# line/open-universe

Hardware: AMD Instinct MI355X
Metric: real_time_factor (audio s / wall s), UNIVERSE++ 16 kHz 8-step enhance (higher is better)
Workload: dtype f32; 1 GPU; UNIVERSE++ 16 kHz, 8 diffusion steps, batch=1 utterance(s) of 4 s per GPU per step; network=PP16, n_diffusion_steps=8, batch_per_gpu=1, samples_per_utterance=64000, launches_per_enhance=414

## Files before the change

### open-universe_amd/csrc/ou_api.cpp

```cpp
#include <hip/hip_runtime.h>

#include <cmath>
#include <cstdio>
#include <cstdlib>
#include <cstring>
#include <map>
#include <string>
#include <vector>

#include "../../include/ouniverse.h"
#include "../../include/ouniverse_tuning.h"
#include "ou_kernels.h"
#include "ou_model.h"

using namespace ou;

namespace {
thread_local std::string g_last_error;
constexpr int kMaxSteps = 256;
constexpr size_t kProfSlots = 32768;
constexpr float kInvSqrt2 = 0.70710678118654752440f;
constexpr size_t align256(size_t bytes) { return (bytes + 255) & ~size_t(255); }

struct TensorRef {
  size_t off;
  int C, T;
};
struct Options {
  int dbg = 0, xcd_map = -1, conv_direct = 5, fuse = -1, fuse_nc = 0, rate_small = 1, fuse_upfir = 1, block3 = 0, d4_fir = 1,
      d4_force = 0, d4_short = 1, d2_wk = 0, wino = 1, d2_map = -1, unfuse64 = 0, preact = 1;
  int gru_v = 2, gru_bmax = 0, gru_ts = 0, gru_upw = 0, gru_backoff = 0, gru_agent = -1, gru_dbg = 0;
  int split = -1;
  int dbg_dec0_under_gru = 0;
  int tile_prefetch = 1;
  int trace = 0, no_overlap = 0, ts = 0, deep_factor = 8, mask_fused = 1, split_wino = 1, d2_tile_rule = 1;
  int ens_share = 1;
  double tile_min = -1.0;
  std::string chain_ts;
};
}

struct ou_packer {
  Model m;
  std::map<std::string, HostTensor> sd;
  std::vector<float> blob;
  std::string err;
};

struct ou_handle {
  Model m;
  const float* W = nullptr;
  int device = 0;
  int num_cu = 256;
  std::string err;
  std::map<std::string, TensorRef> tensors;
  int n_launch = 0, n_conv = 0;
  int cond_B = 0, cond_T = 0;
  bool trace = false;
  Options opt;
  NormMode norm;
  std::string plan_with_options;
  int last_cfg = -1;
  long long* tstamps = nullptr;
  std::map<size_t, float> alphas;
  hipStream_t aux[3] = {nullptr, nullptr, nullptr};
  std::vector<hipEvent_t> events;
  size_t ev_used = 0;
  bool overlap = true;
  int force_cfg = -1, force_sc = 0;
  bool profile = false;
  struct ProfRec { double flops, bytes; int cfg; };
  std::vector<ProfRec> prof;
  size_t prof_used = 0;
  unsigned long long* prof_dev = nullptr;
  struct WsRec { const void* ws; size_t bytes; int B, T; };
  std::vector<WsRec> ws_ready;
  int gru_agent_stores = 0;
  int lanes = 1, lane = 0;
  int lane_max_b = 0;
  struct NoiseSource {
    bool on = false;
    unsigned long long seed = 0;
    std::vector<unsigned long long> streams;
    float* scratch = nullptr;
    size_t scratch_bytes = 0;
  } noise_src;
  double plane_per_sample = 0.0, wav_plane_per_sample = 0.0;
  bool ws_ok(const void* ws, size_t bytes, int B, int T) const {
    (void)T;
    for (const WsRec& r : ws_ready)
      if (r.ws == ws) return r.B == B && r.bytes <= bytes;
    return false;
  }
};

namespace {

int fail(ou_handle* h, int code, const std::string& msg) {
  if (h) h->err = msg;
  g_last_error = msg;
  return code;
}

struct Tensor {
  float* p = nullptr;
  int C = 0, T = 0;
};

struct OptDesc {
  const char* key;
  int Options::*ip;
  double Options::*dp;
  bool experiments_only;
  const char* doc;
};
const OptDesc kOptions[] = {
    {"conv_direct", &Options::conv_direct, nullptr, false, "kernel generations the conv launcher may use (0 .. 5, ConvArgs::direct)"},
    {"split", &Options::split, nullptr, false, "-1 rule / 0 never / 1 wherever possible: conv_split_kernel (bf16-split operands)"},
    {"split_wino", &Options::split_wino, nullptr, false, "experiments build: 0 = the plain bf16-split kernel also where its minimal-filtering form would take the layer"},
    {"wino", &Options::wino, nullptr, false, "0: never the minimal-filtering (Winograd / Cook-Toom) kernel variants"},
    {"fuse", &Options::fuse, nullptr, false, "-1 cost model / 0 never / 2 / 3: depth of the fused ConvBlock body (conv_chain kernels)"},
    {"fuse_nc", &Options::fuse_nc, nullptr, false, "128 / 256: columns per tile of the fused ConvBlock body (0: launcher's choice)"},
    {"fuse_upfir", &Options::fuse_upfir, nullptr, false, "0: up-path anti-alias FIR always as its own pass"},
    {"rate_small", &Options::rate_small, nullptr, false, "0: outermost rate-change convs on the generic kernels (no rate_down / rate_up)"},
    {"preact", &Options::preact, nullptr, false, "0: every PReLU in its consumer's operand path (ConvArgs::out_act never set)"},
    {"unfuse64", &Options::unfuse64, nullptr, false, "1: 64-channel ConvBlock bodies as three split-K launches"},
    {"block3", &Options::block3, nullptr, false, "1: the three body convs of a deep-level ConvBlock in one launch (experiments build only)"},
    {"xcd_map", &Options::xcd_map, nullptr, false, "block -> tile mapping of the LDS-tiled conv kernel (-1: launcher's choice)"},
    {"d2_map", &Options::d2_map, nullptr, false, "block -> tile mapping of the wide-load split-K kernels (-1: launcher's choice)"},
    {"d2_tile_rule", &Options::d2_tile_rule, nullptr, false, "0: round 5's 64- vs 32-column rule of the wide-load split-K kernels (ignores that only 64-column tiles have minimal filtering)"},
    {"d2_wk", &Options::d2_wk, nullptr, false, "4 / 8: K slices of conv_direct2_kernel (0: launcher's rule)"},
    {"d4_fir", &Options::d4_fir, nullptr, false, "0: up convs with a fusable FIR stay on the first-generation fused kernel"},
    {"d4_short", &Options::d4_short, nullptr, false, "0: the 401-frame levels at batch 1 stay on the first-generation kernels"},
    {"d4_force", &Options::d4_force, nullptr, false, "10 TM + log2(WK): that conv_direct4 tile shape wherever a layer admits it"},
    {"tile_min", nullptr, &Options::tile_min, false, "wave tiles per SIMD from which the no-split-K kernels take a layer (< 0: 1.2)"},
    {"tile_prefetch", &Options::tile_prefetch, nullptr, false, "0: no LDS prefetch of the epilogue operand in conv_direct3_kernel"},
    {"deep_factor", &Options::deep_factor, nullptr, false, "blocks of 64 x 128 per CU up to which a layer counts as 'deep' (split-K kernels)"},
    {"mask_fused", &Options::mask_fused, nullptr, false, "ragged batches: 0 = a separate tail-mask launch after EVERY producer (reference form of the masks)"},
    {"gru_v", &Options::gru_v, nullptr, false, "2 ring kernel / 1 polling-wave kernel (experiments build)"},
    {"gru_bmax", &Options::gru_bmax, nullptr, false, "cap on the utterances per GRU launch (forces the chunked path)"},
    {"gru_upw", &Options::gru_upw, nullptr, false, "hidden units per workgroup of the ring kernel (0: from the batch size)"},
    {"gru_backoff", &Options::gru_backoff, nullptr, false, "poll back-off experiments of the ring kernel (0: none)"},
    {"gru_agent_stores", &Options::gru_agent, nullptr, false, "-1 handle's mode / 0 plain / 1 agent-scope publishes"},
    {"gru_dbg", &Options::gru_dbg, nullptr, false, "bit 0 no republish safety net, bit 1 system-scope publishes, bit 2 FAULT INJECTION (tests)"},
    {"gru_ts", &Options::gru_ts, nullptr, false, "1: per-wave cycle stamps of the GRU kernel into the end of the workspace (tuning)"},
    {"ts", &Options::ts, nullptr, false, "1: per-wave phase stamps in ou_bench_conv (tuning)"},
    {"trace", &Options::trace, nullptr, false, "1: one line per conv launch on stderr"},
    {"no_overlap", &Options::no_overlap, nullptr, false, "1: no side streams inside a call (every kernel alone on the device)"},
    {"ens_share", &Options::ens_share, nullptr, false, "ou_enhance_ensemble: 1 = conditioner once over the B inputs, its results replicated; 0 = over all E * B rows"},
    {"dbg", &Options::dbg, nullptr, true, "phase ablation switches of the conv kernels: WRONG results by design"},
    {"dbg_dec0", &Options::dbg_dec0_under_gru, nullptr, true, "first decoder block under the GRU: upper-bound measurement, WRONG results"},
};
constexpr int kNumOptions = (int)(sizeof(kOptions) / sizeof(kOptions[0]));
const OptDesc* find_option(const char* key) {
  for (int i = 0; i < kNumOptions; i++)
    if (std::strcmp(kOptions[i].key, key) == 0) return &kOptions[i];
  return nullptr;
}

struct Runner {
  ou_handle* h;
  Options env;
  char* base;
  size_t cap;
  size_t off = 0;
  bool dry;
  hipStream_t st;
  hipStream_t main_st;
  int B;
  hipError_t herr = hipSuccess;
  bool oom = false;
  const char* where = "";
  size_t max_plane = 0;
  bool mel_scale_preset = false;
  bool ragged = false;
  const int* lens_dev = nullptr;
  const RowInfo* rows_dev = nullptr;
  LevelSpec lv;
  int level_T[kMaxLenLevels] = {0};
  unsigned* status_words = nullptr;
  unsigned long long* block3_bar = nullptr;
  int gru_area_rows = 0;
  bool gru_shared = false;

  Runner(ou_handle* h_, void* ws, size_t cap_, bool dry_, hipStream_t st_, int B_)
      : h(h_), env(h_->opt), base((char*)ws), cap(cap_), dry(dry_), st(st_), main_st(st_), B(B_) {
#ifndef OU_EXPERIMENTS
    env.dbg = 0; env.dbg_dec0_under_gru = 0;
#endif
  }
  static Runner conditioner_of(const Runner& r, int Bc) {
    Runner c(r.h, r.base, r.cap, false, r.st, Bc);
    c.status_words = r.status_words;
    c.block3_bar = r.block3_bar;
    c.gru_area_rows = r.B;
    c.off = r.off;
    c.mel_scale_preset = r.mel_scale_preset;
    c.lv = r.lv;
    for (int l = 0; l < kMaxLenLevels; l++) c.level_T[l] = r.level_T[l];
    return c;
  }
  void set_ragged(const int* lens, const RowInfo* rows) {
    ragged = true;
    lens_dev = lens;
    rows_dev = rows;
  }

  bool ok() const { return herr == hipSuccess && !oom; }
  template <class F>
  void launch(const char* w, F&& enqueue) {
    if (dry || !ok()) return;
    chk(enqueue(), w);
  }

  float* alloc_raw(size_t floats) {
    size_t bytes = align256(floats * 4);
    size_t o = off;
    off += bytes;
    if (!dry && off > cap) { oom = true; return (float*)base; }
    return dry ? nullptr : (float*)(base + o);
  }
  Tensor alloc(const std::string& name, int C, int T) {
    size_t o = off;
    Tensor t;
    t.p = alloc_raw((size_t)B * C * T);
    if ((size_t)C * T * 4 > max_plane) max_plane = (size_t)C * T * 4;
    t.C = C;
    t.T = T;
    if (!name.empty()) h->tensors[name] = TensorRef{o, C, T};
    return t;
  }
  hipEvent_t next_event() {
    if (h->ev_used == h->events.size()) {
      hipEvent_t e;
      if (hipEventCreateWithFlags(&e, hipEventDisableTiming) != hipSuccess) return nullptr;
      h->events.push_back(e);
    }
    return h->events[h->ev_used++];
  }
  void wait_for(hipStream_t from, hipStream_t to, const char* w_record, const char* w_wait) {
    if (dry || !ok()) return;
    hipEvent_t e = next_event();
    if (!e) { herr = hipErrorOutOfMemory; where = "event"; return; }
    launch(w_record, [&] { return hipEventRecord(e, from); });
    launch(w_wait, [&] { return hipStreamWaitEvent(to, e, 0); });
  }
  void fork(hipStream_t from, int k) { wait_for(from, h->aux[k], "fork record", "fork wait"); }
  void join(int k, hipStream_t to) { wait_for(h->aux[k], to, "join record", "join wait"); }
  const int* lens_of(int Tl) {
    if (!ragged) return nullptr;
    for (int l = 0; l < lv.n; l++)
      if (level_T[l] == Tl) return lens_dev + (size_t)l * B;
    if (herr == hipSuccess) { herr = hipErrorInvalidValue; where = "ragged batch: tensor length on no level"; }
    return nullptr;
  }
  void mask(float* p, int C, int T) {
    if (!ragged || dry || !ok()) return;
    const int* ln = lens_of(T);
    if (ln) launch("mask tail", [&] { return launch_mask_tail(p, ln, B, C, T, st); });
  }
  void mask(const Tensor& t) { mask(t.p, t.C, t.T); }
  template <class F>
  void launch_masked(const char* w, float* p, int C, int T, F&& enqueue) {
    const int* ln = env.mask_fused ? lens_of(T) : nullptr;
    launch(w, [&] { return enqueue(ln); });
    if (!ln) mask(p, C, T);
  }
  const float* W(size_t off_floats) const { return h->W + off_floats; }

  unsigned long long* prof_open(double flops, double bytes, int cfg) {
    if (!h->profile || !h->prof_dev || h->prof_used >= kProfSlots) return nullptr;
    h->prof.push_back(ou_handle::ProfRec{flops, bytes, cfg});
    return h->prof_dev + 32 * h->prof_used++;
  }
  void prof_close(const unsigned long long* slot, int cfg) {
    if (slot) h->prof.back().cfg = cfg;
  }
  void prof_drop(const unsigned long long* slot) {
    if (slot) { h->prof.pop_back(); h->prof_used--; }
  }

  struct Epi {
    const float* add = nullptr;
    float add_scale = 1.f;
    const float* film = nullptr;
    int film_bstride = 0;
    const float* res = nullptr;
    float res_scale = 1.f;
    const float* in_scale = nullptr;
    bool act = true;
    const float* fir = nullptr;
    int fir_len = 0;
    const float* fir_bias = nullptr;
    bool rate_down = false;
    bool rate_up = false;
    bool out_act = false;
    float out_alpha = 1.f;
    bool no_mask = false;
  };
  static int gru_share_of(int lanes, int B, bool overlap) {
    const int ncl = 2 * B < 8 ? 2 * B : 8;
    const int by_lanes = lanes > 1 ? (ncl * lanes + 7) / 8 : 1;
    return by_lanes * (overlap ? 2 : 1);
  }

  static int conv_nq(const ConvL& L, int Tin) { return L.stride > 1 ? Tin / L.stride : Tin; }
  static int conv_tout(const ConvL& L, int Tin) { return L.stride > 1 ? Tin / L.stride : Tin * L.up; }
  ConvArgs conv_args(const ConvL& L, const Tensor& in, const Tensor& out, const Epi& e) {
    ConvArgs a;
    a.x = in.p; a.w = W(L.w_off); a.bias = W(L.b_off); a.y = out.p;
    if (L.KWP) { a.wd = W(L.wd_off); a.wu = W(L.wu_off); }
    if (L.ws_on) a.wsplit = W(L.ws_off);
    if (L.wsw_on) a.wsplitw = W(L.wsw_off);
    a.split = env.split; a.split_wino = env.split_wino;
    a.in_scale = e.in_scale;
    a.act = (L.act && e.act) ? 1 : 0;
    a.alpha_val = a.act ? h->alphas[L.a_off] : 0.f;
    a.add = e.add; a.add_scale = e.add_scale;
    a.film = e.film; a.film_bstride = e.film_bstride;
    a.res = e.res; a.res_scale = e.res_scale;
    if (e.out_act && !e.fir && !e.rate_down && !e.rate_up) { a.out_act = 1; a.out_alpha = e.out_alpha; }
    if (e.fir && !e.rate_down) { a.fir = e.fir; a.fir_len = e.fir_len; a.bias = e.fir_bias; }
    if (e.rate_down) { a.fir = e.fir; a.fir_len = e.fir ? e.fir_len : 0; }
    a.B = B; a.Cin = L.Cin; a.Tin = in.T; a.Cout = L.Cout; a.M = L.M; a.Mp = L.Mp; a.KW = L.KW;
    a.stride = L.stride; a.pad = L.pad; a.up = L.up; a.CK = L.CK; a.Nq = conv_nq(L, in.T); a.Tout = conv_tout(L, in.T);
    a.force_cfg = h->force_cfg; a.force_sc = h->force_sc;
    a.dbg = env.dbg; a.force_xcd_map = env.xcd_map; a.direct = env.conv_direct; a.d4_fir_unfused = env.d4_fir; a.d4_force = env.d4_force; a.d4_short = env.d4_short; a.deep_factor = env.deep_factor; a.d2_tile_rule = env.d2_tile_rule; a.d2_wk = env.d2_wk; a.wino = env.wino; a.d2_map = env.d2_map;
    a.tile_min = env.tile_min; a.tile_prefetch = env.tile_prefetch;
    a.tstamps = h->tstamps;
    if (ragged && env.mask_fused && !e.no_mask) a.lens = lens_of(a.Tout);
    return a;
// ... 69 lines not shown
    launch_masked("fir(up)", hu.p, hu.C, hu.T, [&](const int* ln) {
      return launch_fir(u.p, W(rc.fir_off), rc.fir_len, 0.f, 0, W(rc.fbias_off), res, kInvSqrt2, hu.p, B, u.C, u.T, st, ln);
    });
    return hu;
  }

  ChainArgs chain_args(const BlockL& Bk, int depth, const Tensor& hu, const Tensor& c1, const Tensor& v, const Epi& e1,
                       bool need_c1) {
    ChainArgs ca;
    ca.depth = depth; ca.B = B; ca.C = Bk.C; ca.T = hu.T; ca.Mp = Bk.c1.Mp;
    ca.x = depth == 3 ? hu.p : c1.p;
    ca.y = v.p; ca.res = hu.p; ca.res_scale = kInvSqrt2;
    if (depth == 3) {
      ca.add = e1.add; ca.add_scale = e1.add_scale; ca.film = e1.film; ca.film_bstride = e1.film_bstride;
      ca.c1_out = need_c1 ? c1.p : nullptr;
    }
    const ConvL* ls[3] = {&Bk.c1, &Bk.c2, &Bk.c3};
    for (int s2 = 0; s2 < depth; s2++) {
      const ConvL& L = *ls[3 - depth + s2];
      if (!L.act || L.stride != 1 || L.up != 1 || L.Cin != Bk.C || L.Cout != Bk.C || L.pad != (L.KW - 1) / 2 || L.Mp != Bk.c1.Mp)
        ca.depth = 0;
      ChainConv& c = ca.cv[s2];
      c.w = W(L.w_off); c.bias = W(L.b_off); c.alpha = L.act ? h->alphas[L.a_off] : 0.f; c.KW = L.KW; c.CK = L.CK;
      if (L.KWP) c.wu = W(L.wu_off);
    }
    ca.force_nc = env.fuse_nc;
    ca.wino = env.wino && env.conv_direct >= 5;
    ca.lens = lens_of(hu.T);
    return ca;
  }
  int plan_chain(const BlockL& Bk, const Tensor& hu, const Tensor& c1, const Tensor& v, const Epi& e1, bool need_c1) {
    const int T = hu.T;
    if (env.fuse == 0) return 0;
    if (!Bk.all_prelu()) return 0;
    if (ragged && !env.mask_fused) return 0;
    if (env.fuse < 0 && Bk.C % 16 == 0 && Bk.c1.KWP && Bk.c2.KWP && Bk.c3.KWP) {
      if (env.conv_direct >= 3 && direct3_tiles_per_simd(Bk.C, T, B, h->num_cu) >= 1.9 && T >= 1024) return 0;
      if (env.unfuse64 && env.conv_direct >= 5 && env.wino && Bk.C % 64 == 0 && T >= 1024) return 0;
    }
    auto generic = [&](const ConvL& L) {
      const double cyc = 2.0 * L.M * (double)T * L.Cin * L.KW * B / 45e12 * 2.3e9;
      return cyc > 28000.0 ? cyc : 28000.0;
    };
    const double c3 = chain_cost(chain_args(Bk, 3, hu, c1, v, e1, need_c1), h->num_cu, nullptr);
    double c2 = chain_cost(chain_args(Bk, 2, hu, c1, v, e1, need_c1), h->num_cu, nullptr);
    if (c2 >= 0) c2 += generic(Bk.c1);
    if (env.fuse == 3) return c3 >= 0 ? 3 : 0;
    if (env.fuse == 2) return c2 >= 0 ? 2 : 0;
    const double c0 = generic(Bk.c1) + generic(Bk.c2) + generic(Bk.c3);
    int best = 0;
    double bc = c0;
    if (c3 >= 0 && c3 < bc) { best = 3; bc = c3; }
    if (c2 >= 0 && c2 < bc) { best = 2; bc = c2; }
    return best;
  }
  bool body_block3(const BlockL& Bk, const Tensor& hu, const Tensor& c1, const Tensor& c2, const Tensor& v, const std::string& nm,
                   const Epi& e1, const Epi& e3) {
    if (dry || !ok() || env.block3 == 0 || !Bk.all_prelu() || B != 1 || ragged || st != main_st || !block3_bar || h->profile || h->tstamps ||
        h->force_cfg >= 0 || env.conv_direct < 2)
      return false;
    const ConvArgs cv[3] = {conv_args(Bk.c1, hu, c1, e1), conv_args(Bk.c2, c1, c2, Epi()), conv_args(Bk.c3, c2, v, e3)};
    int cfg = -1;
    const hipError_t le = launch_conv_block3(cv, block3_bar, status_words, h->num_cu, st, &cfg);
    if (le == hipErrorInvalidConfiguration) return false;
    if (le != hipSuccess) { launch(nm.c_str(), [le] { return le; }); return false; }
    h->last_cfg = cfg;
    h->n_conv++;
    if (h->trace) std::fprintf(stderr, "OU_TRACE block3 %-62s cfg=%d C=%d T=%d\n", nm.c_str(), cfg, Bk.C, hu.T);
    return true;
  }
  Tensor activated(const ConvL& L, const Tensor& in, const Tensor& plane) {
    if (L.act_kind != OU_ACT_SNAKE && L.act_kind != OU_ACT_SNAKEBETA) return in;
    Tensor s = plane;
    s.C = in.C; s.T = in.T;
    const Model& m = h->m;
    const int* ln = lens_of(in.T);
    launch("snake", [&] {
      return launch_snake_act(in.p, s.p, B, in.C, in.T, in.T, ln, nullptr, W(L.sa_off), L.sb_off != L.sa_off ? W(L.sb_off) : nullptr,
                              W(m.snake_up_off), W(m.snake_down_off), st);
    });
    return s;
  }
  void body(const BlockL& Bk, const Tensor& hu, const Tensor& c1, const Tensor& c2, const Tensor& v, const std::string& nm,
            Epi e1, bool need_c1, bool c1_private, const Tensor& act = Tensor()) {
    const int depth = dry ? 0 : plan_chain(Bk, hu, c1, v, e1, need_c1);
    if (depth == 3 || depth == 2) {
      if (depth == 2) conv(Bk.c1, hu, nm + ".c1", e1, &c1);
      if (!ok()) return;
      ChainArgs ca = chain_args(Bk, depth, hu, c1, v, e1, need_c1);
      if (!env.chain_ts.empty() && nm == env.chain_ts) ca.tstamps = (long long*)(base + cap - (16u << 20));
      double flops = 0, wbytes = 0;
      for (int s2 = 0; s2 < depth; s2++) {
        flops += 2.0 * Bk.C * (double)hu.T * Bk.C * ca.cv[s2].KW * B;
        wbytes += 4.0 * Bk.C * Bk.C * ca.cv[s2].KW;
      }
      ca.prof = prof_open(flops, 4.0 * B * (double)Bk.C * hu.T * (2 + (depth == 2 ? 1 : 0) + (ca.add ? 1 : 0)) + wbytes, -1);
      int variant = -1;
      launch(nm.c_str(), [&] { return launch_chain(ca, h->num_cu, st, &variant); });
      prof_close(ca.prof, variant);
      if (h->trace)
        std::fprintf(stderr, "OU_TRACE chain %-63s variant=%d depth=%d C=%d T=%d B=%d\n", nm.c_str(), variant, depth, Bk.C, hu.T, B);
      h->n_conv++;
      return;
    }
    Epi e3;
    e3.res = dry ? nullptr : hu.p; e3.res_scale = kInvSqrt2;
    if (body_block3(Bk, hu, c1, c2, v, nm, e1, e3)) return;
    if (env.preact && c1_private && Bk.c2.act) { e1.out_act = true; e1.out_alpha = h->alphas[Bk.c2.a_off]; }
    Epi e2;
    e2.act = !conv(Bk.c1, activated(Bk.c1, hu, act), nm + ".c1", e1, &c1).stored_act;
    if (env.preact && Bk.c3.act) { e2.out_act = true; e2.out_alpha = h->alphas[Bk.c3.a_off]; }
    e3.act = !conv(Bk.c2, activated(Bk.c2, c1, act), nm + ".c2", e2, &c2).stored_act;
    conv(Bk.c3, activated(Bk.c3, c2, act), nm + ".v", e3, &v);
  }

  Tensor down_path(const BlockL& Bk, const Tensor& v, const std::string& nm) {
    if (Bk.dir != 1) return v;
    const ConvL& rc = Bk.rc;
    Epi e;
    if (rc.fir_mode <= 1 && env.rate_small != 0 && rate_down_supported(rate_probe(rc, v.T))) {
      e.rate_down = true;
      if (rc.fir_mode == 1) { e.fir = W(rc.fir_off); e.fir_len = rc.fir_len; }
      return conv(rc, v, nm + ".h", e).out;
    }
    if (rc.fir_mode != 1) return conv(rc, v, nm + ".h", e).out;
    const Tensor xf = alloc(nm + ".fir", v.C, v.T);
    launch("fir(down)", [&] {
      return launch_fir(v.p, W(rc.fir_off), rc.fir_len, h->alphas[rc.a_off], 1, nullptr, nullptr, 1.f, xf.p, B, v.C, v.T, st);
    });
    e.act = false;
    return conv(rc, xf, nm + ".h", e).out;
  }

  struct BlockOut { Tensor h_next, v, c1; };
  BlockOut block(const BlockL& Bk, const Tensor& hin, const std::string& nm, const float* film, int film_bs,
                 const float* input_cond, const float* res, bool need_c1 = false, const Tensor* c1_dst = nullptr,
                 const Tensor* v_dst = nullptr) {
    const Tensor hu = up_path(Bk, hin, nm, res);
    Epi e1;
    if (input_cond) { e1.add = input_cond; e1.add_scale = kInvSqrt2; }
    e1.film = film; e1.film_bstride = film_bs;
    BlockOut o;
    o.c1 = c1_dst ? *c1_dst : alloc(nm + ".c1", Bk.c1.Cout, hu.T);
    const Tensor c2 = alloc(nm + ".c2", Bk.c2.Cout, hu.T);
    o.v = v_dst ? *v_dst : alloc(nm + ".v", Bk.c3.Cout, hu.T);
    const Tensor act = Bk.has_snake() ? alloc(nm + ".act", Bk.C, hu.T) : Tensor();
    body(Bk, hu, o.c1, c2, o.v, nm, e1, need_c1, !need_c1 && !c1_dst, act);
    o.h_next = down_path(Bk, o.v, nm);
    return o;
  }

  Tensor gru(const GruL& G, const Tensor& in, const std::string& nm, unsigned long long* xchg, unsigned* errw,
             unsigned* epoch, const float* res, float res_scale, hipEvent_t* before = nullptr) {
    Epi e;
    e.act = false;
    e.no_mask = true;
    Tensor gx = conv(G.proj, in, nm + ".gx", e).out;
    Tensor out = alloc(nm, 2 * G.H, in.T);
    if (dry || !ok()) return out;
    if (const int* ln = lens_of(in.T)) launch("gru tail fill", [&] { return launch_gru_tail_fill(gx.p, ln, B, G.H, in.T, st); });
    GruArgs a;
    a.gx = gx.p; a.whh = W(G.whh_off); a.bhn = W(G.bhn_off); a.out = out.p; a.res = res; a.res_scale = res_scale;
    a.xchg = xchg; a.err = errw; a.epoch = epoch; a.B = B; a.T = in.T; a.H = G.H;
    if (gru_area_rows > B) a.xchg_granules = gru_granules(gru_area_rows, G.H);
    a.version = env.gru_v;
    a.lanes = h->lanes;
    const int Bl = (h->lanes > 1 && h->lane_max_b > B) ? h->lane_max_b : B;
    a.share = gru_share_of(h->lanes, Bl, gru_shared);
    a.xcd_rot = h->lanes > 1 ? (2 * Bl * h->lane) % 8 : 0;
    a.force_bmax = env.gru_bmax;
    if (env.gru_ts) a.tstamps = (long long*)(base + cap - (1u << 20));
    a.force_upw = env.gru_upw;
    a.poll_backoff = env.gru_backoff;
    a.agent_stores = env.gru_agent >= 0 ? (env.gru_agent != 0) : h->gru_agent_stores;
    a.dbg = env.gru_dbg;
    a.prof = prof_open(2.0 * 2.0 * 3.0 * G.H * G.H * (double)in.T * B,
                       4.0 * ((double)B * (6.0 + 2.0 + (res ? 2.0 : 0.0)) * G.H * in.T + 2.0 * 3.0 * G.H * G.H), 1000 + in.T);
    if (before && (*before = next_event())) launch("pre-gru record", [&] { return hipEventRecord(*before, st); });
    launch(G.name.c_str(), [&] { return launch_gru(a, h->num_cu, st); });
    mask(out);
    return out;
  }

 private:
  void chk(hipError_t e, const char* w) {
    if (e != hipSuccess && herr == hipSuccess) { herr = e; where = w; }
    h->n_launch++;
  }
};

struct Persist {
  unsigned* status;
  StepCoef* coef;
  float* stats;
  RowInfo* rows;
  int* lens;
  unsigned long long* xchg;
  unsigned long long* xchg2;
  float* mel_scale;
  float* g;
  float* film;
  Tensor mixn, x, wav;
  std::vector<Tensor> sc;
  std::vector<Tensor> cond;
  Tensor aux, latent;
};

Persist layout_persist(Runner& r, int T) {
  const Model& m = r.h->m;
  Persist P;
  P.status = (unsigned*)r.alloc_raw(64 + 8 * 40 * 2);
  r.status_words = P.status;
  r.block3_bar = (unsigned long long*)(P.status + 64);
  int ncoef = kMaxSteps > r.B ? kMaxSteps : r.B;
  P.coef = (StepCoef*)r.alloc_raw((size_t)ncoef * 8);
  r.h->tensors["stats"] = TensorRef{r.off, 4, 1};
  P.stats = r.alloc_raw((size_t)r.B * 4);
  P.rows = (RowInfo*)r.alloc_raw((size_t)r.B * 4);
  P.lens = (int*)r.alloc_raw((size_t)r.B * kMaxLenLevels);
  P.xchg = (unsigned long long*)r.alloc_raw(gru_granules(r.B, m.OC / 2) * 2);
  P.xchg2 = (unsigned long long*)r.alloc_raw(gru_granules(r.B, m.OC / 2) * 2);
  r.h->tensors["mel_scale"] = TensorRef{r.off, 1, 1};
  P.mel_scale = r.alloc_raw(r.B);
  r.h->tensors["sigma.g"] = TensorRef{r.off, m.film.D, 1};
  P.g = r.alloc_raw((size_t)ncoef * m.film.D);
  r.h->tensors["sigma.film"] = TensorRef{r.off, m.film.rows, 1};
  P.film = r.alloc_raw((size_t)ncoef * m.film.rows);
  P.mixn = r.alloc("mixn", 1, T);
  P.x = r.alloc("x", 1, T);
  P.wav = r.alloc("wav", 1, T);
  for (int j = 0; j < m.n_blocks; j++) {
    const BlockL& b = m.c_dec[j];
    int Tj = T / m.tot_ds;
    int up = 1;
    for (int k = 0; k <= j; k++) if (m.c_dec[k].dir == 2) up *= m.c_dec[k].rate;
    Tj *= up;
    P.cond.push_back(r.alloc("cond.c" + std::to_string(j), b.C, Tj));
    P.sc.push_back(r.alloc("cond.sc" + std::to_string(j), b.C, Tj));
  }
  P.aux = r.alloc("cond.aux", m.C0, T);
  P.latent = r.alloc("cond.latent", m.OC, T / m.tot_ds);
  return P;
}

void run_condition(Runner& r, Persist& P, const float* mix_norm, int T) {
  const Model& m = r.h->m;
  const int L = T / m.tot_ds;
  const int n = m.n_levels - 1;
  hipStream_t main = r.st;
  const bool ov = r.h->overlap && !r.dry && r.h->lanes <= 1;
  if (ov) { r.fork(main, 0); r.st = r.h->aux[0]; }
  Tensor mel = r.alloc("cond.mel", m.mel.n_mels, L);
  float* esum = r.alloc_raw((size_t)r.B * L);
  r.launch("mel", [&] {
    return launch_mel(mix_norm, r.W(m.mel.win_off), r.W(m.mel.tw_off), r.W(m.mel.fb_off), mel.p, esum, r.B, T, m.mel.n_fft,
                      m.mel.hop, m.mel.pad_left, m.mel.n_freq, m.mel.n_mels, L, r.st);
  });
  if (!r.mel_scale_preset) r.launch("mel_scale", [&] { return launch_mel_scale(esum, P.mel_scale, r.B, L, r.st, r.lens_of(L)); });
  r.mask(mel);
  Runner::Epi em;
  em.in_scale = P.mel_scale;
  em.act = false;
  Tensor m0 = r.conv(m.c_melconv, mel, "cond.melconv", em).out;
  Tensor x_mel = r.block(m.c_melblock, m0, "cond.melblock", nullptr, 0, nullptr, nullptr).v;
  r.st = main;
  Tensor e0 = r.alloc("cond.in", m.C0, T);
  r.launch_masked("cond.in", e0.p, e0.C, e0.T, [&](const int* ln) {
    return launch_in_conv(mix_norm, r.W(m.c_in.w_off), r.W(m.c_in.b_off), nullptr, 0, e0.p, r.B, m.C0, T, m.c_in.KW, r.st, ln);
  });
  Tensor hcur = e0;
  std::vector<Tensor> outs;
  for (int i = 0; i < m.n_blocks; i++) {
    auto bo = r.block(m.c_enc[i], hcur, "cond.enc" + std::to_string(i), nullptr, 0, nullptr, nullptr);
    if (i < n - 1) {
      if (ov) { r.fork(main, 1); r.st = r.h->aux[1]; }
      const ConvL& S = m.c_st[i];
      const int R = S.rate, C = S.Cin / R;
      Tensor sd = r.alloc("cond.s2d" + std::to_string(i), S.Cin, bo.v.T / R);
      r.launch("s2d", [&] { return launch_s2d(bo.v.p, r.W(S.a_off), sd.p, r.B, C, bo.v.T, R, r.st); });
      Runner::Epi es;
      es.act = false;
      outs.push_back(r.conv(S, sd, "cond.st" + std::to_string(i), es).out);
      r.st = main;
    }
    hcur = bo.h_next;
  }
  outs.push_back(hcur);
  if (ov) { r.join(0, main); r.join(1, main); }
  Tensor sum = r.alloc("cond.enc_sum", m.OC, L);
  if (!r.dry && r.ok() && outs.size() > 4) { r.herr = hipErrorInvalidValue; r.where = "too many encoder outputs"; return; }
  r.launch("enc_sum", [&] {
    const float* q[4] = {nullptr, nullptr, nullptr, nullptr};
    for (size_t i = 0; i < outs.size(); i++) q[i] = outs[i].p;
    return launch_sum(x_mel.p, q[0], q[1], q[2], q[3], 1.0f / std::sqrt((float)(outs.size() + 1)), sum.p, (size_t)r.B * m.OC * L,
                      r.st);
  });
  Tensor cb1 = r.block(m.c_cb1, sum, "cond.cb1", nullptr, 0, nullptr, nullptr).v;
  Tensor g0 = r.gru(m.c_gru0, cb1, "cond.gru0", P.xchg, P.status, P.status + 2, nullptr, 1.f);
  const bool gres = m.cfg.cond.encoder_gru_residual != 0;
  Tensor g1 = r.gru(m.c_gru1, g0, "cond.gru", P.xchg, P.status, P.status + 2, gres ? cb1.p : nullptr, kInvSqrt2);
  Tensor lat = r.block(m.c_cb2, g1, "cond.cb2", nullptr, 0, nullptr, nullptr, false, nullptr, &P.latent).v;
  Tensor y = r.block(m.c_decin, lat, "cond.decin", nullptr, 0, nullptr, nullptr).v;
  for (int j = 0; j < m.n_blocks; j++) {
    auto bo = r.block(m.c_dec[j], y, "cond.dec" + std::to_string(j), nullptr, 0, nullptr, nullptr, true, &P.cond[j],
                      j == m.n_blocks - 1 ? &P.aux : nullptr);
    y = bo.v;
    {
      Runner::Epi es;
      es.act = false;
      r.conv(m.s_sig[j], bo.c1, "cond.sc" + std::to_string(j), es, &P.sc[j]);
    }
  }
}

struct ScoreEnc {
  std::vector<Tensor> residuals;
  Tensor hg;
  bool fuse_res = false;
};
ScoreEnc run_score_enc(Runner& r, Persist& P, const float* x, const StepCoef* coef, int coef_bs,
                       const float* film_row, int film_bs, int T, hipEvent_t* pre_gru = nullptr) {
  const Model& m = r.h->m;
  ScoreEnc E;
  Tensor e0 = r.alloc("score.in", m.C0, T);
  r.launch_masked("score.in", e0.p, e0.C, e0.T, [&](const int* ln) {
    return launch_in_conv(x, r.W(m.s_in.w_off), r.W(m.s_in.b_off), coef, coef_bs, e0.p, r.B, m.C0, T, m.s_in.KW, r.st, ln);
  });
  Tensor hcur = e0;
  for (int i = 0; i < m.n_blocks; i++) {
    const float* fr = film_row ? film_row + m.film.enc_off[i] : nullptr;
    auto bo = r.block(m.s_enc[i], hcur, "score.enc" + std::to_string(i), fr, film_bs, nullptr, nullptr);
    E.residuals.push_back(bo.v);
    hcur = bo.h_next;
  }
  E.fuse_res = m.s_dec[0].dir == 0;
  E.hg = r.gru(m.s_gru, hcur, "score.gru", P.xchg2, P.status, P.status + 4,
               E.fuse_res && !r.dry ? E.residuals[m.n_blocks - 1].p : nullptr, kInvSqrt2, pre_gru);
  return E;
}
void run_score_dec(Runner& r, Persist& P, const ScoreEnc& E, const float* x, const float* noise, float* out, int mode,
                   const StepCoef* coef, int coef_bs, const float* film_row, int film_bs, int T, const Tensor* dec0_done = nullptr) {
  const Model& m = r.h->m;
  Tensor y = E.hg;
  for (int j = 0; j < m.n_blocks; j++) {
    if (j == 0 && dec0_done) { y = *dec0_done; continue; }
    const float* fr = film_row ? film_row + m.film.dec_off[j] : nullptr;
    const Tensor& res = E.residuals[m.n_blocks - 1 - j];
    const float* resp = (j == 0 && E.fuse_res) ? nullptr : res.p;
    auto bo = r.block(m.s_dec[j], y, "score.dec" + std::to_string(j), fr, film_bs, P.sc[j].p, resp);
    y = bo.v;
  }
  r.launch_masked("score.out", out, 1, T, [&](const int* ln) {
    return launch_out_conv(y.p, r.W(m.s_out.w_off), r.W(m.s_out.b_off), r.W(m.s_out.a_off), x, noise, out, coef, coef_bs,
                           m.cfg.has_edm, mode, r.B, m.C0, T, m.s_out.KW, r.st, ln);
  });
}
static bool m_blocks_ok(const Runner& r) { return r.h->m.n_blocks >= 1 && r.h->m.s_dec[0].dir == 0; }
void run_score(Runner& r, Persist& P, const float* x, const float* noise, float* out, int mode,
               const StepCoef* coef, int coef_bs, const float* film_row, int film_bs, int T) {
  const bool dec0_under = r.env.dbg_dec0_under_gru != 0 && !r.dry && r.h->overlap && r.h->lanes <= 1 && m_blocks_ok(r);
  hipEvent_t pre_gru = nullptr;
  ScoreEnc E = run_score_enc(r, P, x, coef, coef_bs, film_row, film_bs, T, dec0_under ? &pre_gru : nullptr);
  if (dec0_under && pre_gru && r.ok()) {
    const Model& m = r.h->m;
    hipStream_t main = r.st;
    r.launch("dec0 wait", [&] { return hipStreamWaitEvent(r.h->aux[0], pre_gru, 0); });
    r.st = r.h->aux[0];
    const float* fr = film_row ? film_row + m.film.dec_off[0] : nullptr;
    const Tensor& res = E.residuals[m.n_blocks - 1];
    auto bo = r.block(m.s_dec[0], E.hg, "score.dec0", fr, film_bs, P.sc[0].p, E.fuse_res ? nullptr : res.p);
    r.st = main;
    r.join(0, main);
    Tensor done = bo.v;
    run_score_dec(r, P, E, x, noise, out, mode, coef, coef_bs, film_row, film_bs, T, &done);
    return;
  }
  run_score_dec(r, P, E, x, noise, out, mode, coef, coef_bs, film_row, film_bs, T);
}

StepCoef make_coef(const ou_config& cfg, float s, bool last, double eta, double beta, float s_next) {
  StepCoef c;
  const float s2 = s * s;
  if (cfg.has_edm) {
    const double sd = std::pow(10.0, (double)(cfg.has_edm_data_level ? cfg.edm_data_level_db : cfg.level_db) / 20.0);
    const float sd2 = (float)(sd * sd);
    const float sn2 = s2 + sd2;
    const float sn = std::sqrt(sn2);
    c.w_skip = sd2 / sn2;
    c.w_in = 1.0f / sn;
    c.w_out = (s * (float)sd) / sn;
    c.sigma_net = cfg.edm_noise * s;
  } else {
    c.w_skip = 0.f; c.w_in = 1.f; c.w_out = 1.f; c.sigma_net = s;
  }
  c.sig2 = s2;
  c.c1 = last ? s2 : s2 * (float)eta;
  c.s_next = s_next;
  c.beta = (float)beta;
  return c;
}

void schedule(const ou_config& cfg, int n_steps, double epsilon, float* sigma, double* eta, double* beta) {
  const double ratio = (double)cfg.sigma_max / (double)cfg.sigma_min;
  const double delta_t = 1.0 / (n_steps - 1);
  const double gamma = std::pow(ratio, -delta_t);
  *eta = 1.0 - std::pow(gamma, epsilon);
  *beta = std::sqrt(1.0 - std::pow(gamma, 2.0 * (epsilon - 1.0)));
  const float step = 1.0f / (float)(n_steps - 1);
  for (int n = 0; n < n_steps; n++) {
    int i = n_steps - 1 - n;
    float t = (i < n_steps / 2) ? (float)i * step : 1.0f - (float)(n_steps - 1 - i) * step;
    sigma[n] = (float)cfg.sigma_min * std::pow((float)ratio, t);
  }
}

void upload_coefs(Runner& r, StepCoef* dst, const std::vector<StepCoef>& rows) {
  for (size_t i = 0; i < rows.size(); i += 64) {
    CoefBlock blk;
    int n = (int)std::min<size_t>(64, rows.size() - i);
    for (int k = 0; k < n; k++) blk.c[k] = rows[i + k];
    r.launch("upload coef", [&] { return launch_upload_coef(dst + i, blk, n, r.st); });
  }
}

void upload_film_rows(Runner& r, Persist& P, int n) {
  const Model& m = r.h->m;
  r.launch("sigma", [&] { return launch_sigma_embed(P.coef, n, r.W(m.sigma.p_off), m.sigma.simple, m.sigma.n_rff, m.film.D, P.g, r.st); });
  r.launch("film", [&] { return launch_film(P.g, r.W(m.film.w_off), r.W(m.film.b_off), P.film, n, m.film.rows, m.film.D, r.st); });
}

long long max_walk_length(ou_handle* h, bool need_wav);

// ... 421 lines not shown
  }
  int n_steps() const { return (int)sigma.size(); }
  void upload_coef(Runner& r, Persist& P) const { upload_coefs(r, P.coef, coef); }
  void upload_film(Runner& r, Persist& P) const {
    upload_film_rows(r, P, n_steps());
  }
  void upload(Runner& r, Persist& P) const { upload_coef(r, P); upload_film(r, P); }
};

int set_levels(Runner& r, int T) {
  const Model& m = r.h->m;
  LevelSpec& lv = r.lv;
  lv.n = 0;
  auto add_level = [&](int num, int den) {
    lv.num[lv.n] = num; lv.den[lv.n] = den; r.level_T[lv.n] = (int)((long long)T * num / den); lv.n++;
  };
  add_level(1, 1);
  add_level(2, 1);
  int cum = 1;
  for (int i = 0; i < m.cfg.score.n_rates && lv.n < kMaxLenLevels; i++) { cum *= m.cfg.score.rate_factors[i]; add_level(1, cum); }
  if (cum != m.tot_ds) return fail(r.h, OU_EINVAL, "internal: rate factors do not multiply to the total down-sampling factor");
  return OU_OK;
}
void upload_row_lengths(Runner& r, RowInfo* rows_dst, int* lens_dst, const int32_t* t_raw, int n) {
  for (int off = 0; off < n; off += 64) {
    RowBlock blk;
    const int k = n - off < 64 ? n - off : 64;
    for (int i = 0; i < 64; i++) blk.t_raw[i] = i < k ? t_raw[off + i] : 1;
    r.launch("upload rows", [&] { return launch_upload_rows(rows_dst, lens_dst, blk, k, off, n, r.h->m.tot_ds, r.lv, r.st); });
  }
}

void normalize(Runner& r, Persist& P, const float* mix, int rows, int T_raw, int T) {
  const float level = (float)std::pow(10.0, (double)r.h->m.cfg.level_db / 20.0);
  const NormMode nm = r.h->norm;
  r.launch("normalize", [&] {
    return r.ragged ? launch_pad_normalize_var(mix, P.mixn.p, P.stats, P.rows, rows, T_raw, T, level, nm, r.st)
                    : launch_pad_normalize(mix, P.mixn.p, P.stats, rows, T_raw, T, (T - T_raw) / 2, level, nm, r.st);
  });
}
struct PostFlags {
  int keep_rms, peak;
  explicit PostFlags(uint32_t flags) : keep_rms((flags & OU_ENH_KEEP_RMS) ? 1 : 0), peak((flags & OU_ENH_NO_PEAK_GUARD) ? 0 : 1) {}
};
void post(Runner& r, Persist& P, const float* x, float* out, int rows, int T_raw, int T, PostFlags f) {
  r.launch("post", [&] {
    return r.ragged ? launch_post_var(x, P.stats, out, P.rows, rows, T_raw, T, f.keep_rms, f.peak, r.st)
                    : launch_post(x, P.stats, out, rows, T_raw, T, (T - T_raw) / 2, f.keep_rms, f.peak, r.st);
  });
}
void decouple(Runner& r, Persist& P) {
  const Model& m = r.h->m;
  const int T = P.wav.T;
  float* tmp = r.alloc_raw((size_t)r.B * m.C0 * 2 * T);
  r.launch("decoupling", [&] {
    return launch_decoupling(P.aux.p, r.W(m.dec.alpha_off), r.W(m.dec.up_off), r.W(m.dec.down_off), r.W(m.dec.conv.w_off),
                             r.W(m.dec.conv.b_off), tmp, P.wav.p, r.B, m.C0, T, r.st, r.lens_of(T), r.lens_of(2 * T));
  });
}

auto row_noise(Runner& r, const float* noise, int n_start, int T, const int32_t* t_raw) {
  return [&r, noise, n_start, T, t_raw](int draw) -> const float* {
    const ou_handle::NoiseSource& src = r.h->noise_src;
    const size_t nBT = (size_t)r.B * T;
    if (!src.on) return noise + (size_t)(draw ? draw - n_start : 0) * nBT;
    float* dst = src.scratch + (size_t)(draw & 1) * nBT;
    const int tot = r.h->m.tot_ds;
    fill_noise_plane(r, dst, T, r.B, src.seed, draw, [&](int b, unsigned long long& sid, long long& t0, long long& len) {
      sid = src.streams[b];
      t0 = 0;
      len = t_raw ? t_raw[b] + (tot - t_raw[b] % tot) : T;
    });
    return dst;
  };
}

void init_x(Runner& r, Persist& P, const float* z0, const float* warm, float sigma, int T, bool mask) {
  r.launch("init x", [&] { return launch_init_x(z0, warm, sigma, P.x.p, (size_t)r.B * T, r.st); });
  if (mask) r.mask(P.x);
}
struct FirstPass {
  ScoreEnc E;
  size_t off_after_enc = 0;
};
template <typename NoiseFn>
void sample(Runner& r, Persist& P, int T, const SamplerTables& tab, int n_start, const float* warm, bool mask_x0, NoiseFn z,
            const FirstPass* first = nullptr) {
  const Model& m = r.h->m;
  const int n_steps = tab.n_steps();
  if (!first) init_x(r, P, z(0), warm, tab.sigma[n_start], T, mask_x0);
  const size_t step_mark = r.off;
  for (int n = n_start; n < n_steps; n++) {
    const float* zn = n == n_steps - 1 ? nullptr : z(n + 1);
    const StepCoef* cf = P.coef + n;
    const float* fr = P.film + (size_t)n * m.film.rows;
    if (first && n == n_start) {
      r.join(2, r.st);
      r.off = first->off_after_enc;
      run_score_dec(r, P, first->E, P.x.p, zn, P.x.p, OUT_UPDATE, cf, 0, fr, 0, T);
    } else {
      r.off = step_mark;
      run_score(r, P, P.x.p, zn, P.x.p, OUT_UPDATE, cf, 0, fr, 0, T);
    }
    if (!r.ok()) break;
  }
}

int enhance_impl(ou_handle* h, const float* mix, float* out, const float* noise, int32_t B, int32_t T_raw,
                 const int32_t* t_raw, int32_t n_steps, double epsilon, const float* sigma_host, int32_t warm_start,
                 uint32_t flags, void* ws, size_t ws_bytes, ou_stream_t stream) {
  if (!h || !mix || !out || !ws || B < 1 || T_raw < 1) return fail(h, OU_EINVAL, "bad argument");
  if (t_raw)
    if (const int rc = check_rows(h, "ou_enhance_var", 'b', t_raw, B, T_raw, true)) return rc;
  const bool use_aux = (flags & OU_ENH_USE_AUX_SIGNAL) != 0;
  const bool counter = h->noise_src.on;
  if (const int rc = check_noise_source(h, noise, B, "the rows of the call (", !use_aux)) return rc;
  if (const int rc = check_steps(h, n_steps, warm_start)) return rc;
  const Model& m = h->m;
  const int T = T_raw + (m.tot_ds - T_raw % m.tot_ds);
  const bool need_wav = use_aux || warm_start >= 0;
  if (const int rc = check_walk_length(h, T_raw, T, need_wav, "; ou_enhance_segments enhances it in windows")) return rc;
  if (!h->ws_ok(ws, ws_bytes, B, T))
    return fail(h, OU_EINVAL, "workspace was not prepared by ou_workspace_init for this (B, T_raw + pad)");
  if (counter && !use_aux)
    if (const int rc = check_noise_scratch(h, B, T, "ou_noise_scratch_bytes")) return rc;
  CallScope scope(h, (flags & OU_ENH_SERIAL) || h->lanes > 1);
  hipStream_t st = (hipStream_t)stream;
  Runner r(h, ws, ws_bytes, false, st, B);
  Persist P = layout_persist(r, T);
  if (r.oom) return finish(h, r);

  const SamplerTables tab(m.cfg, n_steps, epsilon, sigma_host);
  tab.upload_coef(r, P);
  if (t_raw) {
    if (const int rc = set_levels(r, T)) return rc;
    upload_row_lengths(r, P.rows, P.lens, t_raw, B);
    r.set_ragged(P.lens, P.rows);
  }
  if (need_wav && (!m.dec.present || m.dec.act != OU_ACT_SNAKE))
    return fail(h, OU_ENOTIMPL, "aux_to_wav needs the snake signal-decoupling layer (UNIVERSE++)");
  const int n_start = warm_start >= 0 ? warm_start : 0;
  auto z = row_noise(r, noise, n_start, T, t_raw);

  size_t mark;
  {
    auto keep = h->tensors;
    Runner d(h, nullptr, 0, true, nullptr, B);
    Persist Pd = layout_persist(d, T);
    run_condition(d, Pd, nullptr, T);
    mark = d.off;
    h->tensors = keep;
  }

  FirstPass first;
  bool have_first = false;
  if (!use_aux) {
    tab.upload_film(r, P);
    const int share2 = Runner::gru_share_of(h->lanes, B, true);
    const bool gru_fit = gru_ring_batch_cap(m.s_gru.H, h->num_cu, share2, 0, B, h->lanes) >= 1 &&
                         gru_ring_batch_cap(m.c_gru0.H, h->num_cu, share2, 0, B, h->lanes) >= 1;
    if (warm_start < 0 && h->overlap && gru_fit) {
      r.gru_shared = true;
      init_x(r, P, z(0), nullptr, tab.sigma[n_start], T, true);
      const size_t save = r.off;
      r.fork(st, 2);
      normalize(r, P, mix, B, T_raw, T);
      r.st = h->aux[2];
      r.off = mark;
      first.E = run_score_enc(r, P, P.x.p, P.coef + n_start, 0, P.film + (size_t)n_start * m.film.rows, 0, T);
      first.off_after_enc = r.off;
      r.st = st;
      r.off = save;
      have_first = true;
    }
  }
  if (!have_first) normalize(r, P, mix, B, T_raw, T);
  run_condition(r, P, P.mixn.p, T);
  r.gru_shared = false;
  if (!r.dry && r.ok() && r.off != mark) return fail(h, OU_EINVAL, "internal: workspace layout mismatch");
  h->cond_B = r.ragged ? 0 : B;
  h->cond_T = T;

  if (need_wav) decouple(r, P);
  if (use_aux) {
    post(r, P, P.wav.p, out, B, T_raw, T, PostFlags(flags));
    return finish(h, r);
  }
  sample(r, P, T, tab, n_start, warm_start >= 0 ? P.wav.p : nullptr, true, z, have_first ? &first : nullptr);
  post(r, P, P.x.p, out, B, T_raw, T, PostFlags(flags));
  return finish(h, r);
}
}

extern "C" {

int ou_enhance(ou_handle* h, const float* mix, float* out, const float* noise, int32_t B, int32_t T_raw, int32_t n_steps,
               double epsilon, const float* sigma_host, int32_t warm_start, uint32_t flags, void* ws, size_t ws_bytes,
               ou_stream_t stream) {
  return enhance_impl(h, mix, out, noise, B, T_raw, nullptr, n_steps, epsilon, sigma_host, warm_start, flags, ws, ws_bytes,
                      stream);
}

int ou_enhance_var(ou_handle* h, const float* mix, float* out, const float* noise, int32_t B, int32_t T_raw_max,
                   const int32_t* t_raw, int32_t n_steps, double epsilon, const float* sigma_host, int32_t warm_start,
                   uint32_t flags, void* ws, size_t ws_bytes, ou_stream_t stream) {
  if (!t_raw) return fail(h, OU_EINVAL, "ou_enhance_var: t_raw must be given (ou_enhance takes batches of equal lengths)");
  return enhance_impl(h, mix, out, noise, B, T_raw_max, t_raw, n_steps, epsilon, sigma_host, warm_start, flags, ws, ws_bytes,
                      stream);
}

}

namespace {
struct EnsArea {
  size_t lens_b, members, hist, total;
};
EnsArea ens_area(int B, int E, long long cols) {
  EnsArea a;
  size_t off = 0;
  a.lens_b = off; off += align256((size_t)B * kMaxLenLevels * 4);
  a.members = off; off += align256((size_t)E * B * (size_t)cols * 4);
  a.hist = off; off += align256(((size_t)B * E + B) * 4);
  a.total = off;
  return a;
}

class Replicator {
  Runner& r;
  const int E;
  ReplicateTable tab;
  int n = 0;

 public:
  Replicator(Runner& r_, int E_) : r(r_), E(E_) {}
  void add(void* p, size_t words) {
    if (n == kReplicateEntries) flush();
    tab.p[n] = (unsigned*)p;
    tab.n[n] = (long long)words;
    n++;
  }
  void add(const Tensor& t, int rows) { add(t.p, (size_t)rows * t.C * t.T); }
  void flush() {
    if (n) r.launch("replicate rows", [&] { return launch_replicate_rows(tab, n, E, r.st); });
    n = 0;
  }
};
void replicate_conditioned(Runner& r, Persist& P, int rows, int E, bool with_stats, bool with_wav) {
  Replicator rep(r, E);
  for (size_t j = 0; j < P.cond.size(); j++) { rep.add(P.cond[j], rows); rep.add(P.sc[j], rows); }
  rep.add(P.aux, rows);
  rep.add(P.latent, rows);
  rep.add(P.mixn, rows);
  if (with_stats) rep.add(P.stats, (size_t)rows * 4);
  rep.add(P.mel_scale, (size_t)rows);
  if (with_wav) rep.add(P.wav, rows);
  rep.flush();
}

int ensemble_impl(ou_handle* h, const float* mix, float* out, float* members_out, const float* noise, int32_t B, int32_t T_raw,
                  const int32_t* t_raw, int32_t E, int32_t stat, int32_t n_steps, double epsilon, const float* sigma_host,
// ... 1172 lines not shown
```

Before: 609.7 x_realtime.

## Overlap first score-decoder pass with conditioner via per-level sc events

The first diffusion step's score decoder now runs on side stream 2. Each decoder block waits only on an event recorded after the conditioner produces that level's sc tensor, not on the whole conditioner. This lets decoder levels start while later conditioner levels are still computing, which shortens the critical path of the first step. It adds per-level event records and waits, plus cross-stream hazards on shared workspace, and can be turned off with dec_overlap=0.

Measured after the change: 615.4 x_realtime, median of 6. About the same (+0.9%).

```diff
diff --git a/open-universe_amd/csrc/ou_api.cpp b/open-universe_amd/csrc/ou_api.cpp
--- a/open-universe_amd/csrc/ou_api.cpp
+++ b/open-universe_amd/csrc/ou_api.cpp
@@ -34,6 +34,7 @@
   int dbg_dec0_under_gru = 0;
   int tile_prefetch = 1;
   int trace = 0, no_overlap = 0, ts = 0, deep_factor = 8, mask_fused = 1, split_wino = 1, d2_tile_rule = 1;
+  int dec_overlap = 1;
   int ens_share = 1;
   double tile_min = -1.0;
   std::string chain_ts;
@@ -147,6 +148,7 @@
     {"ts", &Options::ts, nullptr, false, "1: per-wave phase stamps in ou_bench_conv (tuning)"},
     {"trace", &Options::trace, nullptr, false, "1: one line per conv launch on stderr"},
     {"no_overlap", &Options::no_overlap, nullptr, false, "1: no side streams inside a call (every kernel alone on the device)"},
+    {"dec_overlap", &Options::dec_overlap, nullptr, false, "ou_enhance / ou_enhance_var: 1 = the first score-decoder pass on side stream 2, each level behind the conditioner's sc of that level; 0 = behind the whole conditioner"},
     {"ens_share", &Options::ens_share, nullptr, false, "ou_enhance_ensemble: 1 = conditioner once over the B inputs, its results replicated; 0 = over all E * B rows"},
     {"dbg", &Options::dbg, nullptr, true, "phase ablation switches of the conv kernels: WRONG results by design"},
     {"dbg_dec0", &Options::dbg_dec0_under_gru, nullptr, true, "first decoder block under the GRU: upper-bound measurement, WRONG results"},
@@ -247,6 +249,22 @@
   }
   void fork(hipStream_t from, int k) { wait_for(from, h->aux[k], "fork record", "fork wait"); }
   void join(int k, hipStream_t to) { wait_for(h->aux[k], to, "join record", "join wait"); }
+  void join_always(int k, hipStream_t to) {
+    if (ok()) { join(k, to); return; }
+    if (dry) return;
+    hipEvent_t e = next_event();
+    if (e && hipEventRecord(e, h->aux[k]) == hipSuccess) (void)hipStreamWaitEvent(to, e, 0);
+  }
+  hipEvent_t record_here(const char* w) {
+    if (dry || !ok()) return nullptr;
+    hipEvent_t e = next_event();
+    if (!e) { herr = hipErrorOutOfMemory; where = "event"; return nullptr; }
+    launch(w, [&] { return hipEventRecord(e, st); });
+    return e;
+  }
+  void wait_here(hipEvent_t e, const char* w) {
+    if (e) launch(w, [&] { return hipStreamWaitEvent(st, e, 0); });
+  }
   const int* lens_of(int Tl) {
     if (!ragged) return nullptr;
     for (int l = 0; l < lv.n; l++)
@@ -482,9 +500,10 @@
     return s;
   }
   void body(const BlockL& Bk, const Tensor& hu, const Tensor& c1, const Tensor& c2, const Tensor& v, const std::string& nm,
-            Epi e1, bool need_c1, bool c1_private, const Tensor& act = Tensor()) {
+            Epi e1, bool need_c1, bool c1_private, const Tensor& act = Tensor(), hipEvent_t add_ready = nullptr) {
     const int depth = dry ? 0 : plan_chain(Bk, hu, c1, v, e1, need_c1);
     if (depth == 3 || depth == 2) {
+      wait_here(add_ready, "cond wait");
       if (depth == 2) conv(Bk.c1, hu, nm + ".c1", e1, &c1);
       if (!ok()) return;
       ChainArgs ca = chain_args(Bk, depth, hu, c1, v, e1, need_c1);
@@ -505,10 +524,12 @@
     }
     Epi e3;
     e3.res = dry ? nullptr : hu.p; e3.res_scale = kInvSqrt2;
+    const Tensor in1 = activated(Bk.c1, hu, act);
+    wait_here(add_ready, "cond wait");
     if (body_block3(Bk, hu, c1, c2, v, nm, e1, e3)) return;
     if (env.preact && c1_private && Bk.c2.act) { e1.out_act = true; e1.out_alpha = h->alphas[Bk.c2.a_off]; }
     Epi e2;
-    e2.act = !conv(Bk.c1, activated(Bk.c1, hu, act), nm + ".c1", e1, &c1).stored_act;
+    e2.act = !conv(Bk.c1, in1, nm + ".c1", e1, &c1).stored_act;
     if (env.preact && Bk.c3.act) { e2.out_act = true; e2.out_alpha = h->alphas[Bk.c3.a_off]; }
     e3.act = !conv(Bk.c2, activated(Bk.c2, c1, act), nm + ".c2", e2, &c2).stored_act;
     conv(Bk.c3, activated(Bk.c3, c2, act), nm + ".v", e3, &v);
@@ -535,7 +556,7 @@
   struct BlockOut { Tensor h_next, v, c1; };
   BlockOut block(const BlockL& Bk, const Tensor& hin, const std::string& nm, const float* film, int film_bs,
                  const float* input_cond, const float* res, bool need_c1 = false, const Tensor* c1_dst = nullptr,
-                 const Tensor* v_dst = nullptr) {
+                 const Tensor* v_dst = nullptr, hipEvent_t cond_ready = nullptr) {
     const Tensor hu = up_path(Bk, hin, nm, res);
     Epi e1;
     if (input_cond) { e1.add = input_cond; e1.add_scale = kInvSqrt2; }
@@ -545,7 +566,7 @@
     const Tensor c2 = alloc(nm + ".c2", Bk.c2.Cout, hu.T);
     o.v = v_dst ? *v_dst : alloc(nm + ".v", Bk.c3.Cout, hu.T);
     const Tensor act = Bk.has_snake() ? alloc(nm + ".act", Bk.C, hu.T) : Tensor();
-    body(Bk, hu, o.c1, c2, o.v, nm, e1, need_c1, !need_c1 && !c1_dst, act);
+    body(Bk, hu, o.c1, c2, o.v, nm, e1, need_c1, !need_c1 && !c1_dst, act, cond_ready);
     o.h_next = down_path(Bk, o.v, nm);
     return o;
   }
@@ -643,12 +664,17 @@
   return P;
 }
 
-void run_condition(Runner& r, Persist& P, const float* mix_norm, int T) {
+struct CondReady {
+  std::vector<hipEvent_t> sc;
+};
+
+void run_condition(Runner& r, Persist& P, const float* mix_norm, int T, CondReady* ready = nullptr) {
   const Model& m = r.h->m;
   const int L = T / m.tot_ds;
   const int n = m.n_levels - 1;
   hipStream_t main = r.st;
   const bool ov = r.h->overlap && !r.dry && r.h->lanes <= 1;
+  if (ready) ready->sc.assign(m.n_blocks, nullptr);
   if (ov) { r.fork(main, 0); r.st = r.h->aux[0]; }
   Tensor mel = r.alloc("cond.mel", m.mel.n_mels, L);
   float* esum = r.alloc_raw((size_t)r.B * L);
@@ -709,6 +735,7 @@
       Runner::Epi es;
       es.act = false;
       r.conv(m.s_sig[j], bo.c1, "cond.sc" + std::to_string(j), es, &P.sc[j]);
+      if (ready) ready->sc[j] = r.record_here("sc ready record");
     }
   }
 }
@@ -739,7 +766,8 @@
   return E;
 }
 void run_score_dec(Runner& r, Persist& P, const ScoreEnc& E, const float* x, const float* noise, float* out, int mode,
-                   const StepCoef* coef, int coef_bs, const float* film_row, int film_bs, int T, const Tensor* dec0_done = nullptr) {
+                   const StepCoef* coef, int coef_bs, const float* film_row, int film_bs, int T, const Tensor* dec0_done = nullptr,
+                   const CondReady* sc_ready = nullptr) {
   const Model& m = r.h->m;
   Tensor y = E.hg;
   for (int j = 0; j < m.n_blocks; j++) {
@@ -747,7 +775,8 @@
     const float* fr = film_row ? film_row + m.film.dec_off[j] : nullptr;
     const Tensor& res = E.residuals[m.n_blocks - 1 - j];
     const float* resp = (j == 0 && E.fuse_res) ? nullptr : res.p;
-    auto bo = r.block(m.s_dec[j], y, "score.dec" + std::to_string(j), fr, film_bs, P.sc[j].p, resp);
+    auto bo = r.block(m.s_dec[j], y, "score.dec" + std::to_string(j), fr, film_bs, P.sc[j].p, resp, false, nullptr, nullptr,
+                      sc_ready ? sc_ready->sc[j] : nullptr);
     y = bo.v;
   }
   r.launch_masked("score.out", out, 1, T, [&](const int* ln) {
@@ -1335,6 +1364,7 @@
 struct FirstPass {
   ScoreEnc E;
   size_t off_after_enc = 0;
+  const CondReady* sc_ready = nullptr;
 };
 template <typename NoiseFn>
 void sample(Runner& r, Persist& P, int T, const SamplerTables& tab, int n_start, const float* warm, bool mask_x0, NoiseFn z,
@@ -1344,9 +1374,20 @@
   if (!first) init_x(r, P, z(0), warm, tab.sigma[n_start], T, mask_x0);
   const size_t step_mark = r.off;
   for (int n = n_start; n < n_steps; n++) {
-    const float* zn = n == n_steps - 1 ? nullptr : z(n + 1);
     const StepCoef* cf = P.coef + n;
     const float* fr = P.film + (size_t)n * m.film.rows;
+    if (first && n == n_start && first->sc_ready) {
+      hipStream_t main = r.st;
+      r.st = r.h->aux[2];
+      const float* zn = n == n_steps - 1 ? nullptr : z(n + 1);
+      r.off = first->off_after_enc;
+      run_score_dec(r, P, first->E, P.x.p, zn, P.x.p, OUT_UPDATE, cf, 0, fr, 0, T, nullptr, first->sc_ready);
+      r.st = main;
+      r.join_always(2, main);
+      if (!r.ok()) break;
+      continue;
+    }
+    const float* zn = n == n_steps - 1 ? nullptr : z(n + 1);
     if (first && n == n_start) {
       r.join(2, r.st);
       r.off = first->off_after_enc;
@@ -1428,7 +1469,14 @@
     }
   }
   if (!have_first) normalize(r, P, mix, B, T_raw, T);
-  run_condition(r, P, P.mixn.p, T);
+  CondReady sc_ready;
+  const bool dec_beside = have_first && r.env.dec_overlap != 0;
+  run_condition(r, P, P.mixn.p, T, dec_beside ? &sc_ready : nullptr);
+  if (dec_beside && r.ok()) {
+    for (hipEvent_t e : sc_ready.sc)
+      if (!e) { r.herr = hipErrorInvalidValue; r.where = "a signal-condition tensor without its event"; }
+  }
+  if (dec_beside) first.sc_ready = &sc_ready;
   r.gru_shared = false;
   if (!r.dry && r.ok() && r.off != mark) return fail(h, OU_EINVAL, "internal: workspace layout mismatch");
   h->cond_B = r.ragged ? 0 : B;
```
